# LuoweiZhou/VLP

Measured on NVIDIA H100. Metric: image_text_samples_per_sec, higher is better.
Workload: dtype bf16

## Files before the change

vlp_b200/csrc/api.cu:

```cuda
#include "../../include/vlpk.h"

#include <cstdlib>
#include <cstring>

#include "attn.cuh"
#include "gemm.cuh"
#include "head.cuh"
#include "host.cuh"
#include "optim.cuh"
#include "rowops.cuh"
#include "tables.cuh"

using namespace vlpk;
typedef __nv_bfloat16 bf16;

namespace {

inline cudaStream_t S(void* s) { return reinterpret_cast<cudaStream_t>(s); }

enum { SITE_ATTN = 0, SITE_HID1 = 1, SITE_HID2 = 2 };
inline uint64_t site_of(uint64_t layer_id, int site) { return layer_id * 8 + site; }

inline DropoutCfg mk_drop(const VlpkDropout* d, float p, uint64_t site) {
  if (d == nullptr || p <= 0.f) return make_dropout(0.f, 0, site);
// ... 324 lines not shown
    o[j] = pack_bf16x2(v.x > 0.f ? d.x * scale : 0.f, v.y > 0.f ? d.y * scale : 0.f);
  }
  *reinterpret_cast<uint4*>(dpre + i) = make_uint4(o[0], o[1], o[2], o[3]);
}

}

#pragma GCC visibility push(default)
extern "C" {

int vlpk_version(void) { return VLPK_VERSION; }
int vlpk_debug_set_option(const char* name, int value) {
  VLPK_CHECK_ARG(name != nullptr, "set_option: null name");
  if (strcmp(name, "wgrad_stream") == 0) { g_wgrad_stream = value ? 1 : 0; return 0; }
  if (strcmp(name, "attn_tiled") == 0) { set_attn_tiled(value != 0); return 0; }
  set_error("set_option: unknown option '%s'", name);
  return -1;
}
int vlpk_debug_plan_gemm(int M, int N, int K, int a_mn, int b_mn, int nseg, int seg_rows, int epi, int bn, int splits, int* out2) {
  GemmDesc g;
  g.M = M; g.N = N; g.K = K;
  g.a_mn = a_mn != 0; g.b_mn = b_mn != 0;
  g.nseg = nseg; g.b_seg_rows = seg_rows;
  g.epi = epi; g.bn = bn; g.splits = splits;
  return plan_gemm(g, &out2[0], &out2[1]);
}
void vlpk_set_reserved_sms(int n) { set_reserved_sms(n); }
void vlpk_set_deterministic(int on) { set_deterministic(on != 0); }
const char* vlpk_last_error(void) { return get_error(); }

// ... 405 lines not shown
```

vlp_b200/csrc/attn.cu:

```cuda
#include "attn.cuh"
#include "host.cuh"
#include "rowops.cuh"

namespace vlpk {

static constexpr int HD = 64;
static constexpr int TL = 128;
static constexpr int TILE_B = TL * 128;
static constexpr float LOG2E = 1.4426950408889634f;
static constexpr float LN2 = 0.6931471805599453f;
static constexpr int ATT_THREADS = 256;

struct AttnTmaps {
  CUtensorMap q, k, v, o;
  CUtensorMap dq, dk, dv;
};

struct AttnArgs {
  int B, heads, Lq, Lkv;
  const uint32_t* mask_bits;
  int mask_rows;
  float* lse;
  const __nv_bfloat16* o_ptr;
  const __nv_bfloat16* do_ptr;
// ... 13 lines not shown
    const int t = threadIdx.x & 127, lane = threadIdx.x & 31;
    fr = (t >> 5) * 16 + (lane >> 2);
    fc = (lane & 3) * 2;
  }
};

__device__ __forceinline__ float quad_max(float v) {
  v = fmaxf(v, __shfl_xor_sync(0xffffffffu, v, 1));
  return fmaxf(v, __shfl_xor_sync(0xffffffffu, v, 2));
}
__device__ __forceinline__ float quad_sum(float v) {
  v += __shfl_xor_sync(0xffffffffu, v, 1);
  return v + __shfl_xor_sync(0xffffffffu, v, 2);
}

__device__ __forceinline__ void attn_keep_words(const DropoutCfg& d, uint64_t dseed, const uint64_t (&row_elem0)[2], uint32_t (&kw)[2][4]) {
  const int lane = threadIdx.x & 31, qi = lane & 3;
#pragma unroll
  for (int h = 0; h < 2; ++h) {
    uint32_t mine = 0xFFFFFFFFu;
    if (d.p > 0.f) {
      if (d.bits != nullptr) {
        mine = __ldg(reinterpret_cast<const uint32_t*>(d.bits + (row_elem0[h] >> 3)) + qi);
      } else {
        mine = 0;
#pragma unroll
        for (int g = 0; g < 4; ++g) mine |= dropout_keep8(dseed, d.site, (row_elem0[h] + qi * 32 + g * 8) >> 3, d.thresh16) << (8 * g);
      }
    }
#pragma unroll
    for (int w = 0; w < 4; ++w) kw[h][w] = __shfl_sync(0xffffffffu, mine, (lane & ~3) | w);
  }
}

__device__ __forceinline__ float score(float s, const uint32_t (&mw)[4], int col, int Lkv) {
  const float x = s * (0.125f * LOG2E) + (((mw[col >> 5] >> (col & 31)) & 1u) ? 0.f : -10000.0f * LOG2E);
  return col < Lkv ? x : -INFINITY;
}

__device__ __forceinline__ void load_mask_words(const AttnArgs& a, int b, int row, uint32_t (&mw)[4]) {
  const int mr = (a.mask_rows == 1) ? 0 : min(row, a.mask_rows - 1);
  const uint4 m4 = __ldg(reinterpret_cast<const uint4*>(a.mask_bits + (static_cast<size_t>(b) * a.mask_rows + mr) * 4));
  mw[0] = m4.x; mw[1] = m4.y; mw[2] = m4.z; mw[3] = m4.w;
}

struct FwdSmem {
  static constexpr int OFF_Q = 0;
  static constexpr int OFF_K = TILE_B;
  static constexpr int OFF_V = 2 * TILE_B;
  static constexpr int OFF_BAR = 3 * TILE_B;
  static constexpr int TOTAL = OFF_BAR + 16;
  static constexpr int DYN = TOTAL + 1024;
};

__global__ void __launch_bounds__(ATT_THREADS, 2) attn_fwd_kernel(const __grid_constant__ AttnTmaps tm, const AttnArgs a) {
  extern __shared__ uint8_t smem_raw[];
  uint8_t* smem = reinterpret_cast<uint8_t*>((reinterpret_cast<uintptr_t>(smem_raw) + 1023) & ~uintptr_t(1023));
  uint8_t* sQ = smem + FwdSmem::OFF_Q;
  uint8_t* sK = smem + FwdSmem::OFF_K;
  uint8_t* sV = smem + FwdSmem::OFF_V;
  uint64_t* bars = reinterpret_cast<uint64_t*>(smem + FwdSmem::OFF_BAR);
  uint64_t* bar_qk = &bars[0];
  uint64_t* bar_v = &bars[1];

  pdl_launch_dependents();
  const int h = blockIdx.x, b = blockIdx.y;
  const int tid = threadIdx.x, wg = tid >> 7;
  const Frag f;
  const int qi = tid & 3;

  if (tid == 0) {
    tma_prefetch_desc(&tm.q);
    tma_prefetch_desc(&tm.k);
    tma_prefetch_desc(&tm.v);
    tma_prefetch_desc(&tm.o);
    mbar_init(bar_qk, 1);
    mbar_init(bar_v, 1);
    fence_mbar_init();
  }
  __syncthreads();
  pdl_wait();
  if (tid == 0) {
    mbar_arrive_expect_tx(bar_qk, 2 * TILE_B);
    tma_load_3d(sQ, &tm.q, bar_qk, h * HD, 0, b);
    tma_load_3d(sK, &tm.k, bar_qk, h * HD, 0, b);
    mbar_arrive_expect_tx(bar_v, TILE_B);
    tma_load_3d(sV, &tm.v, bar_v, h * HD, 0, b);
  }

  const int row[2] = {wg * 64 + f.fr, wg * 64 + f.fr + 8};
  uint32_t mw[2][4];
  uint64_t row_elem0[2];
#pragma unroll
  for (int hh = 0; hh < 2; ++hh) {
    load_mask_words(a, b, row[hh], mw[hh]);
    row_elem0[hh] = ((static_cast<uint64_t>(b) * a.heads + h) * a.Lq + min(row[hh], a.Lq - 1)) * TL;
  }

  float s[64];
  mbar_wait(bar_qk, 0);
  {
    const uint32_t q0 = smem_u32(sQ) + wg * 8192, k0 = smem_u32(sK);
    wgmma_fence();
#pragma unroll
    for (int k = 0; k < HD / 16; ++k)
      wgmma_m64n128k16_ss<0, 0>(s, wgmma_desc_sw128(q0 + k * 32, 16, 1024), wgmma_desc_sw128(k0 + k * 32, 16, 1024), k > 0 ? 1u : 0u);
    wgmma_commit();
    wgmma_wait<0>();
    reg_fence(s);
  }
  float mx[2] = {-INFINITY, -INFINITY};
#pragma unroll
  for (int i = 0; i < 64; ++i) {
    const int hh = (i >> 1) & 1;
    s[i] = score(s[i], mw[hh], 8 * (i >> 2) + f.fc + (i & 1), a.Lkv);
    mx[hh] = fmaxf(mx[hh], s[i]);
  }
  mx[0] = quad_max(mx[0]);
  mx[1] = quad_max(mx[1]);
  uint32_t kw[2][4];
  attn_keep_words(a.drop, drop_seed(a.drop), row_elem0, kw);
  if (a.keep_out != nullptr) {
#pragma unroll
    for (int hh = 0; hh < 2; ++hh)
      if (row[hh] < a.Lq) reinterpret_cast<uint32_t*>(a.keep_out + (row_elem0[hh] >> 3))[qi] = kw[hh][qi];
  }
  float rsum[2] = {0.f, 0.f}, lsum[2] = {0.f, 0.f};
  uint32_t pa[8][4];
#pragma unroll
  for (int i = 0; i < 64; i += 2) {
    const int hh = (i >> 1) & 1, col = 8 * (i >> 2) + f.fc;
    const float x0 = fast_ex2(s[i] - mx[hh]), x1 = fast_ex2(s[i + 1] - mx[hh]);
    lsum[hh] += x0 + x1;
    const float e0 = bf16_round(x0), e1 = bf16_round(x1);
    rsum[hh] += e0 + e1;
    const uint32_t keep = kw[hh][col >> 5] >> (col & 31);
    const float p0 = (keep & 1u) ? e0 * a.drop.scale : 0.f;
    const float p1 = (keep & 2u) ? e1 * a.drop.scale : 0.f;
    pa[i >> 3][(i >> 1) & 3] = pack_bf16x2(p0, p1);
  }
#pragma unroll
  for (int hh = 0; hh < 2; ++hh) {
    rsum[hh] = quad_sum(rsum[hh]);
    lsum[hh] = quad_sum(lsum[hh]);
    if (qi == 0 && a.lse != nullptr && row[hh] < a.Lq)
      a.lse[(static_cast<size_t>(b) * a.heads + h) * a.Lq + row[hh]] = (mx[hh] + log2f(lsum[hh])) * LN2;
  }
  float o[32];
  mbar_wait(bar_v, 0);
  {
    const uint32_t v0 = smem_u32(sV);
    wgmma_fence();
#pragma unroll
    for (int k = 0; k < TL / 16; ++k) wgmma_m64n64k16_rs<1>(o, pa[k], wgmma_desc_sw128(v0 + k * 2048, 8192, 1024), k > 0 ? 1u : 0u);
    wgmma_commit();
    wgmma_wait<0>();
    reg_fence(o);
  }
  const float inv[2] = {1.0f / rsum[0], 1.0f / rsum[1]};
  uint8_t* stg = sQ + wg * 8192;
#pragma unroll
  for (int i = 0; i < 32; i += 2) {
    const int hh = (i >> 1) & 1;
    sw_write_pair(stg, f.fr + 8 * hh, 8 * (i >> 2) + f.fc, pack_bf16x2(o[i] * inv[hh], o[i + 1] * inv[hh]));
  }
  fence_proxy_async_smem();
  __syncthreads();
  if (tid == 0) {
    tma_store_3d(&tm.o, sQ, h * HD, 0, b);
    tma_store_commit();
    tma_store_wait<0>();
  }
}

struct BwdSmem {
  static constexpr int OFF_Q = 0;
  static constexpr int OFF_K = TILE_B;
  static constexpr int OFF_V = 2 * TILE_B;
  static constexpr int OFF_DO = 3 * TILE_B;
  static constexpr int OFF_PD = 4 * TILE_B;
  static constexpr int OFF_BAR = 6 * TILE_B;
  static constexpr int TOTAL = OFF_BAR + 16;
  static constexpr int DYN = TOTAL + 1024;
};

__global__ void __launch_bounds__(ATT_THREADS, 1) attn_bwd_kernel(const __grid_constant__ AttnTmaps tm, const AttnArgs a) {
  extern __shared__ uint8_t smem_raw[];
  uint8_t* smem = reinterpret_cast<uint8_t*>((reinterpret_cast<uintptr_t>(smem_raw) + 1023) & ~uintptr_t(1023));
  uint8_t* sQ = smem + BwdSmem::OFF_Q;
  uint8_t* sK = smem + BwdSmem::OFF_K;
  uint8_t* sV = smem + BwdSmem::OFF_V;
  uint8_t* sdO = smem + BwdSmem::OFF_DO;
  uint8_t* sPD = smem + BwdSmem::OFF_PD;
  uint64_t* bar_in = reinterpret_cast<uint64_t*>(smem + BwdSmem::OFF_BAR);

  pdl_launch_dependents();
  const int h = blockIdx.x, b = blockIdx.y;
  const int tid = threadIdx.x, wg = tid >> 7;
  const Frag f;

  if (tid == 0) {
    tma_prefetch_desc(&tm.q);
    tma_prefetch_desc(&tm.k);
    tma_prefetch_desc(&tm.v);
    tma_prefetch_desc(&tm.o);
    mbar_init(bar_in, 1);
    fence_mbar_init();
  }
  __syncthreads();
  pdl_wait();
  if (tid == 0) {
    mbar_arrive_expect_tx(bar_in, 4 * TILE_B);
    tma_load_3d(sQ, &tm.q, bar_in, h * HD, 0, b);
    tma_load_3d(sK, &tm.k, bar_in, h * HD, 0, b);
    tma_load_3d(sV, &tm.v, bar_in, h * HD, 0, b);
    tma_load_3d(sdO, &tm.o, bar_in, h * HD, 0, b);
  }

  const int row[2] = {wg * 64 + f.fr, wg * 64 + f.fr + 8};
  uint32_t mw[2][4];
  uint64_t row_elem0[2];
  float lse2[2];
  bool row_ok[2];
#pragma unroll
  for (int hh = 0; hh < 2; ++hh) {
    load_mask_words(a, b, row[hh], mw[hh]);
    row_elem0[hh] = ((static_cast<uint64_t>(b) * a.heads + h) * a.Lq + min(row[hh], a.Lq - 1)) * TL;
    row_ok[hh] = row[hh] < a.Lq;
    lse2[hh] = row_ok[hh] ? a.lse[(static_cast<size_t>(b) * a.heads + h) * a.Lq + row[hh]] * LOG2E : 0.f;
  }
  uint32_t kw[2][4];
  attn_keep_words(a.drop, drop_seed(a.drop), row_elem0, kw);

  float s[64], dp[64];
  mbar_wait(bar_in, 0);
  {
    const uint32_t q0 = smem_u32(sQ) + wg * 8192, k0 = smem_u32(sK), do0 = smem_u32(sdO) + wg * 8192, v0 = smem_u32(sV);
    wgmma_fence();
#pragma unroll
    for (int k = 0; k < HD / 16; ++k)
      wgmma_m64n128k16_ss<0, 0>(s, wgmma_desc_sw128(q0 + k * 32, 16, 1024), wgmma_desc_sw128(k0 + k * 32, 16, 1024), k > 0 ? 1u : 0u);
#pragma unroll
    for (int k = 0; k < HD / 16; ++k)
      wgmma_m64n128k16_ss<0, 0>(dp, wgmma_desc_sw128(do0 + k * 32, 16, 1024), wgmma_desc_sw128(v0 + k * 32, 16, 1024), k > 0 ? 1u : 0u);
    wgmma_commit();
    wgmma_wait<0>();
    reg_fence(s);
    reg_fence(dp);
  }
  float delta[2] = {0.f, 0.f};
#pragma unroll
  for (int i = 0; i < 64; ++i) {
    const int hh = (i >> 1) & 1, col = 8 * (i >> 2) + f.fc + (i & 1);
    const float p = row_ok[hh] ? fast_ex2(score(s[i], mw[hh], col, a.Lkv) - lse2[hh]) : 0.f;
    const bool kp = (kw[hh][col >> 5] >> (col & 31)) & 1u;
    const float dpm = kp ? dp[i] * a.drop.scale : 0.f;
    delta[hh] = fmaf(p, dpm, delta[hh]);
    s[i] = p;
    dp[i] = dpm;
  }
  delta[0] = quad_sum(delta[0]);
  delta[1] = quad_sum(delta[1]);
  uint32_t dsa[8][4];
#pragma unroll
  for (int i = 0; i < 64; i += 2) {
    const int hh = (i >> 1) & 1, col = 8 * (i >> 2) + f.fc;
    const uint32_t keep = kw[hh][col >> 5] >> (col & 31);
    const float p0 = (keep & 1u) ? s[i] * a.drop.scale : 0.f, p1 = (keep & 2u) ? s[i + 1] * a.drop.scale : 0.f;
    sw_write_pair(sPD + (col >> 6) * TILE_B, row[hh], col & 63, pack_bf16x2(p0, p1));
    dsa[i >> 3][(i >> 1) & 3] = pack_bf16x2(s[i] * (dp[i] - delta[hh]) * 0.125f, s[i + 1] * (dp[i + 1] - delta[hh]) * 0.125f);
  }
  fence_proxy_async_smem();
  __syncthreads();

  float dv[32];
  {
    const uint32_t p0 = smem_u32(sPD) + wg * TILE_B, do0 = smem_u32(sdO);
    wgmma_fence();
#pragma unroll
    for (int k = 0; k < TL / 16; ++k)
      wgmma_m64n64k16_ss<1, 1>(dv, wgmma_desc_sw128(p0 + k * 2048, 8192, 1024), wgmma_desc_sw128(do0 + k * 2048, 8192, 1024), k > 0 ? 1u : 0u);
    wgmma_commit();
    wgmma_wait<0>();
    reg_fence(dv);
  }
  __syncthreads();
#pragma unroll
  for (int c = 0; c < 8; ++c)
#pragma unroll
    for (int e = 0; e < 4; ++e) {
      const int hh = e & 1, col = 16 * c + 8 * (e >> 1) + f.fc;
      sw_write_pair(sPD + (col >> 6) * TILE_B, row[hh], col & 63, dsa[c][e]);
    }
  fence_proxy_async_smem();
  __syncthreads();

  float dk[32], dq[32];
  {
    const uint32_t p0 = smem_u32(sPD) + wg * TILE_B, q0 = smem_u32(sQ), k0 = smem_u32(sK);
    wgmma_fence();
#pragma unroll
    for (int k = 0; k < TL / 16; ++k)
      wgmma_m64n64k16_ss<1, 1>(dk, wgmma_desc_sw128(p0 + k * 2048, 8192, 1024), wgmma_desc_sw128(q0 + k * 2048, 8192, 1024), k > 0 ? 1u : 0u);
#pragma unroll
    for (int k = 0; k < TL / 16; ++k) wgmma_m64n64k16_rs<1>(dq, dsa[k], wgmma_desc_sw128(k0 + k * 2048, 8192, 1024), k > 0 ? 1u : 0u);
    wgmma_commit();
    wgmma_wait<0>();
    reg_fence(dk);
    reg_fence(dq);
  }
  __syncthreads();
#pragma unroll
  for (int i = 0; i < 32; i += 2) {
    const int r = wg * 64 + f.fr + 8 * ((i >> 1) & 1), col = 8 * (i >> 2) + f.fc;
    sw_write_pair(sQ, r, col, pack_bf16x2(dq[i], dq[i + 1]));
    sw_write_pair(sK, r, col, pack_bf16x2(dk[i], dk[i + 1]));
    sw_write_pair(sV, r, col, pack_bf16x2(dv[i], dv[i + 1]));
  }
  fence_proxy_async_smem();
  __syncthreads();
  if (tid == 0) {
    tma_store_3d(&tm.dq, sQ, h * HD, 0, b);
    tma_store_3d(&tm.dk, sK, h * HD, 0, b);
    tma_store_3d(&tm.dv, sV, h * HD, 0, b);
    tma_store_commit();
  }
  if (a.dbias_part != nullptr && tid < 192) {
    const int o = tid >> 6, c = tid & 63;
    const uint8_t* stg = (o == 0) ? sQ : (o == 1 ? sK : sV);
    float acc = 0.f;
#pragma unroll 8
    for (int r = 0; r < TL; ++r)
      acc += __bfloat162float(*reinterpret_cast<const __nv_bfloat16*>(stg + r * 128 + (((c >> 3) ^ (r & 7)) << 4) + (c & 7) * 2));
    a.dbias_part[static_cast<size_t>(b) * 3 * a.heads * HD + o * a.heads * HD + h * HD + c] = acc;
  }
  if (tid == 0) tma_store_wait<0>();
}

static constexpr int MAX_SLOTS = 512;
static bool g_attn_tiled = false;

void set_attn_tiled(bool on) { g_attn_tiled = on; }

struct AttnTiledArgs {
  int B, heads, Lq, Lkv;
  int slots;
  int tiles;
  const uint32_t* mask_bits;
  int mask_rows;
  float* lse;
// ... 1 lines not shown
  DropoutCfg drop;
  unsigned char* keep_out;
  float* dbias_part;
};

__device__ __forceinline__ void load_mask_tile(const AttnTiledArgs& a, int b, int row, int kt, uint32_t (&mw)[4]) {
  const int mr = (a.mask_rows == 1) ? 0 : min(row, a.mask_rows - 1);
  const uint4 m4 = __ldg(reinterpret_cast<const uint4*>(a.mask_bits + (static_cast<size_t>(b) * a.mask_rows + mr) * (a.slots >> 5)) + kt);
  mw[0] = m4.x; mw[1] = m4.y; mw[2] = m4.z; mw[3] = m4.w;
}

__device__ __forceinline__ uint64_t tiled_row_elem0(const AttnTiledArgs& a, int b, int h, int row) {
  return ((static_cast<uint64_t>(b) * a.heads + h) * a.Lq + min(row, a.Lq - 1)) * a.slots;
}

__device__ __forceinline__ float staged_colsum(const uint8_t* stg, int c) {
  float acc = 0.f;
#pragma unroll 8
  for (int r = 0; r < TL; ++r)
    acc += __bfloat162float(*reinterpret_cast<const __nv_bfloat16*>(stg + r * 128 + (((c >> 3) ^ (r & 7)) << 4) + (c & 7) * 2));
  return acc;
}

struct FwdTiledSmem {
  static constexpr int OFF_Q = 0;
  static constexpr int OFF_KV = TILE_B;
  static constexpr int OFF_BAR = 5 * TILE_B;
  static constexpr int TOTAL = OFF_BAR + 24;
  static constexpr int DYN = TOTAL + 1024;
};

__global__ void __launch_bounds__(ATT_THREADS, 1) attn_fwd_tiled_kernel(const __grid_constant__ AttnTmaps tm, const AttnTiledArgs a) {
  extern __shared__ uint8_t smem_raw[];
  uint8_t* smem = reinterpret_cast<uint8_t*>((reinterpret_cast<uintptr_t>(smem_raw) + 1023) & ~uintptr_t(1023));
  uint8_t* sQ = smem + FwdTiledSmem::OFF_Q;
  uint8_t* sKV = smem + FwdTiledSmem::OFF_KV;
  uint64_t* bars = reinterpret_cast<uint64_t*>(smem + FwdTiledSmem::OFF_BAR);

// ... 426 lines not shown
  if (d.kv_slots == 0) {
    VLPK_CHECK_ARG(d.Lq >= 1 && d.Lq <= TL && d.Lkv >= 1 && d.Lkv <= TL, "attention: Lq=%d Lkv=%d must be in [1,128]",
                   d.Lq, d.Lkv);
  } else {
    VLPK_CHECK_ARG(d.Lkv >= 1 && d.Lkv <= MAX_SLOTS && d.kv_slots == (d.Lkv + TL - 1) / TL * TL && d.Lq >= 1 && d.Lq <= d.kv_slots,
                   "attention: Lq=%d Lkv=%d kv_slots=%d (needs Lkv in [1,512], kv_slots = 128 * ceil(Lkv / 128), Lq in [1,kv_slots])",
                   d.Lq, d.Lkv, d.kv_slots);
  }
  VLPK_CHECK_ARG(d.B >= 1 && d.heads >= 1, "attention: B=%d heads=%d", d.B, d.heads);
  VLPK_CHECK_ARG(d.mask_bits != nullptr && (d.mask_rows == 1 || d.mask_rows == d.Lq), "attention: mask rows %d",
                 d.mask_rows);
  return 0;
}

static bool use_tiled(const AttnDesc& d) { return g_attn_tiled || d.Lq > TL || d.Lkv > TL; }

static AttnTiledArgs tiled_args(const AttnDesc& d) {
  AttnTiledArgs a;
  a.B = d.B; a.heads = d.heads; a.Lq = d.Lq; a.Lkv = d.Lkv;
  a.slots = d.kv_slots != 0 ? d.kv_slots : TL;
  a.tiles = (d.Lq + TL - 1) / TL;
  a.mask_bits = d.mask_bits; a.mask_rows = d.mask_rows;
  a.lse = d.lse; a.delta = nullptr;
  a.drop = d.drop;
  a.keep_out = nullptr;
  a.dbias_part = nullptr;
  return a;
}

static int launch_attn_fwd_tiled(const AttnDesc& d, const AttnTmaps& tm, cudaStream_t stream) {
// ... 44 lines not shown
  AttnTmaps tm;
  memset(&tm, 0, sizeof(tm));
  VLPK_TRY(make_seq_tmap(&tm.q, d.q, width, d.Lq, d.B, d.ld_q));
  VLPK_TRY(make_seq_tmap(&tm.k, d.k, width, d.Lkv, d.B, d.ld_kv, d.kv_batch_stride));
  VLPK_TRY(make_seq_tmap(&tm.v, d.v, width, d.Lkv, d.B, d.ld_kv, d.kv_batch_stride));
  VLPK_TRY(make_seq_tmap(&tm.o, d.o, width, d.Lq, d.B, d.ld_o));
  tm.dq = tm.dk = tm.dv = tm.o;
  if (use_tiled(d)) return launch_attn_fwd_tiled(d, tm, stream);
  AttnArgs a;
  a.B = d.B; a.heads = d.heads; a.Lq = d.Lq; a.Lkv = d.Lkv;
  a.mask_bits = d.mask_bits; a.mask_rows = d.mask_rows;
  a.lse = d.lse; a.o_ptr = nullptr; a.do_ptr = nullptr; a.ld_o = d.ld_o;
  a.drop = d.drop;
  a.keep_out = d.keep_out;
  a.dbias_part = nullptr;
  static bool attr_set = false;
  if (!attr_set) {
    VLPK_CUDA(cudaFuncSetAttribute(attn_fwd_kernel, cudaFuncAttributeMaxDynamicSharedMemorySize, FwdSmem::DYN));
    attr_set = true;
  }
  LaunchScope scope(CAT_ATTN_FWD, 4.0 * d.B * d.heads * d.Lq * d.Lkv * HD, stream);
  VLPK_CUDA(launch_ex(attn_fwd_kernel, dim3(d.heads, d.B), dim3(ATT_THREADS), FwdSmem::DYN, stream, 1, tm, a));
  return 0;
}

int launch_attn_bwd(const AttnDesc& d, cudaStream_t stream) {
  VLPK_TRY(check_common(d));
  VLPK_CHECK_ARG(d.Lq == d.Lkv, "attention bwd: Lq must equal Lkv (training path)");
  VLPK_CHECK_ARG(d.lse != nullptr && d.d_o != nullptr && d.dq && d.dk && d.dv, "attention bwd: missing buffers");
  const int width = d.heads * HD;
  AttnTmaps tm;
  memset(&tm, 0, sizeof(tm));
  VLPK_TRY(make_seq_tmap(&tm.q, d.q, width, d.Lq, d.B, d.ld_q));
  VLPK_TRY(make_seq_tmap(&tm.k, d.k, width, d.Lkv, d.B, d.ld_kv));
  VLPK_TRY(make_seq_tmap(&tm.v, d.v, width, d.Lkv, d.B, d.ld_kv));
  VLPK_TRY(make_seq_tmap(&tm.o, d.d_o, width, d.Lq, d.B, d.ld_o));
  VLPK_TRY(make_seq_tmap(&tm.dq, d.dq, width, d.Lq, d.B, d.ld_dqkv));
// ... 3 lines not shown
  AttnArgs a;
  a.B = d.B; a.heads = d.heads; a.Lq = d.Lq; a.Lkv = d.Lkv;
  a.mask_bits = d.mask_bits; a.mask_rows = d.mask_rows;
  a.lse = d.lse;
  a.o_ptr = reinterpret_cast<const __nv_bfloat16*>(d.o);
  a.do_ptr = reinterpret_cast<const __nv_bfloat16*>(d.d_o);
  a.ld_o = d.ld_o;
  a.drop = d.drop;
  a.keep_out = nullptr;
  a.dbias_part = nullptr;
  const long long nbias = 3LL * d.heads * HD;
  if (d.dbias != nullptr) {
    a.dbias_part = scratch_f32(SCRATCH_ATTN_DBIAS, static_cast<size_t>(d.B) * nbias, stream);
    if (a.dbias_part == nullptr) return -1;
  }
  static bool attr_set = false;
  if (!attr_set) {
    VLPK_CUDA(cudaFuncSetAttribute(attn_bwd_kernel, cudaFuncAttributeMaxDynamicSharedMemorySize, BwdSmem::DYN));
    attr_set = true;
  }
  {
    LaunchScope scope(CAT_ATTN_BWD, 10.0 * d.B * d.heads * d.Lq * d.Lkv * HD, stream);
    VLPK_CUDA(launch_ex(attn_bwd_kernel, dim3(d.heads, d.B), dim3(ATT_THREADS), BwdSmem::DYN, stream, 1, tm, a));
  }
  if (d.dbias != nullptr) VLPK_TRY(launch_sum_parts(a.dbias_part, d.B, nbias, d.dbias, stream));
  return 0;
}

}
```

vlp_b200/csrc/attn.cuh:

```cuda
#pragma once
#include "common.cuh"

namespace vlpk {

struct AttnDesc {
  int B = 0, heads = 0, head_dim = 64;
  int Lq = 0, Lkv = 0;
  int kv_slots = 0;
  const void* q = nullptr;
  const void* k = nullptr;
  const void* v = nullptr;
  int64_t ld_q = 0, ld_kv = 0;
  int64_t kv_batch_stride = 0;
  void* o = nullptr;
  int64_t ld_o = 0;
  const uint32_t* mask_bits = nullptr;
  int mask_rows = 0;
  float* lse = nullptr;
  DropoutCfg drop = {0.f, 1.f, 0u, 0ull, 0ull, nullptr};
  unsigned char* keep_out = nullptr;
  const void* d_o = nullptr;
  void* dq = nullptr;
  void* dk = nullptr;
  void* dv = nullptr;
  int64_t ld_dqkv = 0;
  float* dbias = nullptr;
};

int launch_attn_fwd(const AttnDesc& d, cudaStream_t stream);
int launch_attn_bwd(const AttnDesc& d, cudaStream_t stream);
void set_attn_tiled(bool on);

}
```

Measured before the change: 4040.

## Make short-sequence attention kernels persistent with double-buffered TMA prefetch

Converts the single-tile attention forward and backward kernels from one CTA per (head, batch) into persistent CTAs sized by occupancy. Each CTA loops over work items and prefetches the next item's Q/K/V(/dO) via TMA into a second stage while computing the current one. The backward pass also overlaps the dbias column sums and the next item's mask/LSE/dropout loads with WGMMA, and mask bit extraction is precomputed with per-fragment shifts. The cost is that the forward shared memory doubles, which may lower occupancy, and the backward kernel adds a separate output staging area.

```diff
diff --git a/vlp_b200/csrc/api.cu b/vlp_b200/csrc/api.cu
--- a/vlp_b200/csrc/api.cu
+++ b/vlp_b200/csrc/api.cu
@@ -362,6 +362,7 @@
   VLPK_CHECK_ARG(name != nullptr, "set_option: null name");
   if (strcmp(name, "wgrad_stream") == 0) { g_wgrad_stream = value ? 1 : 0; return 0; }
   if (strcmp(name, "attn_tiled") == 0) { set_attn_tiled(value != 0); return 0; }
+  if (strcmp(name, "attn_ctas") == 0) { set_attn_ctas(value); return 0; }
   set_error("set_option: unknown option '%s'", name);
   return -1;
 }
diff --git a/vlp_b200/csrc/attn.cu b/vlp_b200/csrc/attn.cu
--- a/vlp_b200/csrc/attn.cu
+++ b/vlp_b200/csrc/attn.cu
@@ -51,29 +51,48 @@
   return v + __shfl_xor_sync(0xffffffffu, v, 2);
 }
 
-__device__ __forceinline__ void attn_keep_words(const DropoutCfg& d, uint64_t dseed, const uint64_t (&row_elem0)[2], uint32_t (&kw)[2][4]) {
-  const int lane = threadIdx.x & 31, qi = lane & 3;
+__device__ __forceinline__ void attn_keep_own(const DropoutCfg& d, uint64_t dseed, const uint64_t (&row_elem0)[2], uint32_t (&mine)[2]) {
+  const int qi = threadIdx.x & 3;
 #pragma unroll
   for (int h = 0; h < 2; ++h) {
-    uint32_t mine = 0xFFFFFFFFu;
+    mine[h] = 0xFFFFFFFFu;
     if (d.p > 0.f) {
       if (d.bits != nullptr) {
-        mine = __ldg(reinterpret_cast<const uint32_t*>(d.bits + (row_elem0[h] >> 3)) + qi);
+        mine[h] = __ldg(reinterpret_cast<const uint32_t*>(d.bits + (row_elem0[h] >> 3)) + qi);
       } else {
-        mine = 0;
-#pragma unroll
-        for (int g = 0; g < 4; ++g) mine |= dropout_keep8(dseed, d.site, (row_elem0[h] + qi * 32 + g * 8) >> 3, d.thresh16) << (8 * g);
+        mine[h] = 0;
+#pragma unroll
+        for (int g = 0; g < 4; ++g) mine[h] |= dropout_keep8(dseed, d.site, (row_elem0[h] + qi * 32 + g * 8) >> 3, d.thresh16) << (8 * g);
       }
     }
-#pragma unroll
-    for (int w = 0; w < 4; ++w) kw[h][w] = __shfl_sync(0xffffffffu, mine, (lane & ~3) | w);
-  }
-}
-
+  }
+}
+__device__ __forceinline__ void attn_keep_share(const uint32_t (&mine)[2], uint32_t (&kw)[2][4]) {
+  const int lane = threadIdx.x & 31;
+#pragma unroll
+  for (int h = 0; h < 2; ++h)
+#pragma unroll
+    for (int w = 0; w < 4; ++w) kw[h][w] = __shfl_sync(0xffffffffu, mine[h], (lane & ~3) | w);
+}
+__device__ __forceinline__ void attn_keep_words(const DropoutCfg& d, uint64_t dseed, const uint64_t (&row_elem0)[2], uint32_t (&kw)[2][4]) {
+  uint32_t mine[2];
+  attn_keep_own(d, dseed, row_elem0, mine);
+  attn_keep_share(mine, kw);
+}
+
+__device__ __forceinline__ float score_bit(float s, uint32_t attend, bool valid) {
+  const float x = s * (0.125f * LOG2E) + (attend ? 0.f : -10000.0f * LOG2E);
+  return valid ? x : -INFINITY;
+}
 __device__ __forceinline__ float score(float s, const uint32_t (&mw)[4], int col, int Lkv) {
-  const float x = s * (0.125f * LOG2E) + (((mw[col >> 5] >> (col & 31)) & 1u) ? 0.f : -10000.0f * LOG2E);
-  return col < Lkv ? x : -INFINITY;
-}
+  return score_bit(s, (mw[col >> 5] >> (col & 31)) & 1u, col < Lkv);
+}
+
+__device__ __forceinline__ void frag_shift(uint32_t (&w)[4], int fc) {
+#pragma unroll
+  for (int j = 0; j < 4; ++j) w[j] >>= fc;
+}
+__device__ __forceinline__ uint32_t frag_bit(const uint32_t (&w)[4], int i) { return (w[i >> 4] >> (8 * ((i >> 2) & 3) + (i & 1))) & 1u; }
 
 __device__ __forceinline__ void load_mask_words(const AttnArgs& a, int b, int row, uint32_t (&mw)[4]) {
   const int mr = (a.mask_rows == 1) ? 0 : min(row, a.mask_rows - 1);
@@ -81,296 +100,349 @@
   mw[0] = m4.x; mw[1] = m4.y; mw[2] = m4.z; mw[3] = m4.w;
 }
 
+static int g_attn_ctas = 0;
+
+void set_attn_ctas(int n) { g_attn_ctas = n > 0 ? n : 0; }
+
 struct FwdSmem {
-  static constexpr int OFF_Q = 0;
-  static constexpr int OFF_K = TILE_B;
-  static constexpr int OFF_V = 2 * TILE_B;
-  static constexpr int OFF_BAR = 3 * TILE_B;
-  static constexpr int TOTAL = OFF_BAR + 16;
+  static constexpr int STAGE = 3 * TILE_B;
+  static constexpr int OFF_BAR = 2 * STAGE;
+  static constexpr int TOTAL = OFF_BAR + 32;
   static constexpr int DYN = TOTAL + 1024;
 };
 
 __global__ void __launch_bounds__(ATT_THREADS, 2) attn_fwd_kernel(const __grid_constant__ AttnTmaps tm, const AttnArgs a) {
   extern __shared__ uint8_t smem_raw[];
   uint8_t* smem = reinterpret_cast<uint8_t*>((reinterpret_cast<uintptr_t>(smem_raw) + 1023) & ~uintptr_t(1023));
-  uint8_t* sQ = smem + FwdSmem::OFF_Q;
-  uint8_t* sK = smem + FwdSmem::OFF_K;
-  uint8_t* sV = smem + FwdSmem::OFF_V;
   uint64_t* bars = reinterpret_cast<uint64_t*>(smem + FwdSmem::OFF_BAR);
-  uint64_t* bar_qk = &bars[0];
-  uint64_t* bar_v = &bars[1];
 
   pdl_launch_dependents();
-  const int h = blockIdx.x, b = blockIdx.y;
   const int tid = threadIdx.x, wg = tid >> 7;
   const Frag f;
   const int qi = tid & 3;
+
+  auto load_item = [&](int w, int st) {
+    const int h = w % a.heads, b = w / a.heads;
+    uint8_t* sq = smem + st * FwdSmem::STAGE;
+    mbar_arrive_expect_tx(&bars[2 * st], 2 * TILE_B);
+    tma_load_3d(sq, &tm.q, &bars[2 * st], h * HD, 0, b);
+    tma_load_3d(sq + TILE_B, &tm.k, &bars[2 * st], h * HD, 0, b);
+    mbar_arrive_expect_tx(&bars[2 * st + 1], TILE_B);
+    tma_load_3d(sq + 2 * TILE_B, &tm.v, &bars[2 * st + 1], h * HD, 0, b);
+  };
 
   if (tid == 0) {
     tma_prefetch_desc(&tm.q);
     tma_prefetch_desc(&tm.k);
     tma_prefetch_desc(&tm.v);
     tma_prefetch_desc(&tm.o);
-    mbar_init(bar_qk, 1);
-    mbar_init(bar_v, 1);
+    for (int i = 0; i < 4; ++i) mbar_init(&bars[i], 1);
     fence_mbar_init();
   }
   __syncthreads();
   pdl_wait();
-  if (tid == 0) {
-    mbar_arrive_expect_tx(bar_qk, 2 * TILE_B);
-    tma_load_3d(sQ, &tm.q, bar_qk, h * HD, 0, b);
-    tma_load_3d(sK, &tm.k, bar_qk, h * HD, 0, b);
-    mbar_arrive_expect_tx(bar_v, TILE_B);
-    tma_load_3d(sV, &tm.v, bar_v, h * HD, 0, b);
-  }
+  if (tid == 0) load_item(blockIdx.x, 0);
 
   const int row[2] = {wg * 64 + f.fr, wg * 64 + f.fr + 8};
-  uint32_t mw[2][4];
-  uint64_t row_elem0[2];
-#pragma unroll
-  for (int hh = 0; hh < 2; ++hh) {
-    load_mask_words(a, b, row[hh], mw[hh]);
-    row_elem0[hh] = ((static_cast<uint64_t>(b) * a.heads + h) * a.Lq + min(row[hh], a.Lq - 1)) * TL;
-  }
-
-  float s[64];
-  mbar_wait(bar_qk, 0);
-  {
-    const uint32_t q0 = smem_u32(sQ) + wg * 8192, k0 = smem_u32(sK);
-    wgmma_fence();
-#pragma unroll
-    for (int k = 0; k < HD / 16; ++k)
-      wgmma_m64n128k16_ss<0, 0>(s, wgmma_desc_sw128(q0 + k * 32, 16, 1024), wgmma_desc_sw128(k0 + k * 32, 16, 1024), k > 0 ? 1u : 0u);
-    wgmma_commit();
+  int it = 0;
+  for (int w = blockIdx.x; w < a.B * a.heads; w += gridDim.x, ++it) {
+    const int st = it & 1;
+    const uint32_t par = (it >> 1) & 1;
+    const int h = w % a.heads, b = w / a.heads;
+    uint8_t* sQ = smem + st * FwdSmem::STAGE;
+    if (tid == 0 && w + static_cast<int>(gridDim.x) < a.B * a.heads) {
+      tma_store_wait_read<0>();
+      load_item(w + gridDim.x, st ^ 1);
+    }
+
+    uint32_t mw[2][4];
+#pragma unroll
+    for (int hh = 0; hh < 2; ++hh) {
+      load_mask_words(a, b, row[hh], mw[hh]);
+      frag_shift(mw[hh], f.fc);
+    }
+
+    float s[64];
+    mbar_wait(&bars[2 * st], par);
+    {
+      const uint32_t q0 = smem_u32(sQ) + wg * 8192, k0 = smem_u32(sQ + TILE_B);
+      wgmma_fence();
+#pragma unroll
+      for (int k = 0; k < HD / 16; ++k)
+        wgmma_m64n128k16_ss<0, 0>(s, wgmma_desc_sw128(q0 + k * 32, 16, 1024), wgmma_desc_sw128(k0 + k * 32, 16, 1024), k > 0 ? 1u : 0u);
+      wgmma_commit();
+    }
+    uint64_t row_elem0[2];
+#pragma unroll
+    for (int hh = 0; hh < 2; ++hh) row_elem0[hh] = (static_cast<uint64_t>(w) * a.Lq + min(row[hh], a.Lq - 1)) * TL;
+    uint32_t mine[2];
+    attn_keep_own(a.drop, drop_seed(a.drop), row_elem0, mine);
     wgmma_wait<0>();
     reg_fence(s);
-  }
-  float mx[2] = {-INFINITY, -INFINITY};
-#pragma unroll
-  for (int i = 0; i < 64; ++i) {
-    const int hh = (i >> 1) & 1;
-    s[i] = score(s[i], mw[hh], 8 * (i >> 2) + f.fc + (i & 1), a.Lkv);
-    mx[hh] = fmaxf(mx[hh], s[i]);
-  }
-  mx[0] = quad_max(mx[0]);
-  mx[1] = quad_max(mx[1]);
-  uint32_t kw[2][4];
-  attn_keep_words(a.drop, drop_seed(a.drop), row_elem0, kw);
-  if (a.keep_out != nullptr) {
-#pragma unroll
-    for (int hh = 0; hh < 2; ++hh)
-      if (row[hh] < a.Lq) reinterpret_cast<uint32_t*>(a.keep_out + (row_elem0[hh] >> 3))[qi] = kw[hh][qi];
-  }
-  float rsum[2] = {0.f, 0.f}, lsum[2] = {0.f, 0.f};
-  uint32_t pa[8][4];
-#pragma unroll
-  for (int i = 0; i < 64; i += 2) {
-    const int hh = (i >> 1) & 1, col = 8 * (i >> 2) + f.fc;
-    const float x0 = fast_ex2(s[i] - mx[hh]), x1 = fast_ex2(s[i + 1] - mx[hh]);
-    lsum[hh] += x0 + x1;
-    const float e0 = bf16_round(x0), e1 = bf16_round(x1);
-    rsum[hh] += e0 + e1;
-    const uint32_t keep = kw[hh][col >> 5] >> (col & 31);
-    const float p0 = (keep & 1u) ? e0 * a.drop.scale : 0.f;
-    const float p1 = (keep & 2u) ? e1 * a.drop.scale : 0.f;
-    pa[i >> 3][(i >> 1) & 3] = pack_bf16x2(p0, p1);
-  }
-#pragma unroll
-  for (int hh = 0; hh < 2; ++hh) {
-    rsum[hh] = quad_sum(rsum[hh]);
-    lsum[hh] = quad_sum(lsum[hh]);
-    if (qi == 0 && a.lse != nullptr && row[hh] < a.Lq)
-      a.lse[(static_cast<size_t>(b) * a.heads + h) * a.Lq + row[hh]] = (mx[hh] + log2f(lsum[hh])) * LN2;
-  }
-  float o[32];
-  mbar_wait(bar_v, 0);
-  {
-    const uint32_t v0 = smem_u32(sV);
-    wgmma_fence();
-#pragma unroll
-    for (int k = 0; k < TL / 16; ++k) wgmma_m64n64k16_rs<1>(o, pa[k], wgmma_desc_sw128(v0 + k * 2048, 8192, 1024), k > 0 ? 1u : 0u);
-    wgmma_commit();
-    wgmma_wait<0>();
-    reg_fence(o);
-  }
-  const float inv[2] = {1.0f / rsum[0], 1.0f / rsum[1]};
-  uint8_t* stg = sQ + wg * 8192;
-#pragma unroll
-  for (int i = 0; i < 32; i += 2) {
-    const int hh = (i >> 1) & 1;
-    sw_write_pair(stg, f.fr + 8 * hh, 8 * (i >> 2) + f.fc, pack_bf16x2(o[i] * inv[hh], o[i + 1] * inv[hh]));
-  }
-  fence_proxy_async_smem();
-  __syncthreads();
-  if (tid == 0) {
-    tma_store_3d(&tm.o, sQ, h * HD, 0, b);
-    tma_store_commit();
-    tma_store_wait<0>();
-  }
+    float mx[2] = {-INFINITY, -INFINITY};
+    const int lim = a.Lkv - f.fc;
+#pragma unroll
+    for (int i = 0; i < 64; ++i) {
+      const int hh = (i >> 1) & 1;
+      s[i] = score_bit(s[i], frag_bit(mw[hh], i), 8 * (i >> 2) + (i & 1) < lim);
+      mx[hh] = fmaxf(mx[hh], s[i]);
+    }
+    mx[0] = quad_max(mx[0]);
+    mx[1] = quad_max(mx[1]);
+    uint32_t kw[2][4];
+    attn_keep_share(mine, kw);
+    frag_shift(kw[0], f.fc);
+    frag_shift(kw[1], f.fc);
+    if (a.keep_out != nullptr) {
+#pragma unroll
+      for (int hh = 0; hh < 2; ++hh)
+        if (row[hh] < a.Lq) reinterpret_cast<uint32_t*>(a.keep_out + (row_elem0[hh] >> 3))[qi] = mine[hh];
+    }
+    float rsum[2] = {0.f, 0.f}, lsum[2] = {0.f, 0.f};
+    uint32_t pa[8][4];
+#pragma unroll
+    for (int i = 0; i < 64; i += 2) {
+      const int hh = (i >> 1) & 1;
+      const float x0 = fast_ex2(s[i] - mx[hh]), x1 = fast_ex2(s[i + 1] - mx[hh]);
+      lsum[hh] += x0 + x1;
+      const float e0 = bf16_round(x0), e1 = bf16_round(x1);
+      rsum[hh] += e0 + e1;
+      const float p0 = frag_bit(kw[hh], i) ? e0 * a.drop.scale : 0.f;
+      const float p1 = frag_bit(kw[hh], i + 1) ? e1 * a.drop.scale : 0.f;
+      pa[i >> 3][(i >> 1) & 3] = pack_bf16x2(p0, p1);
+    }
+#pragma unroll
+    for (int hh = 0; hh < 2; ++hh) {
+      rsum[hh] = quad_sum(rsum[hh]);
+      lsum[hh] = quad_sum(lsum[hh]);
+      if (qi == 0 && a.lse != nullptr && row[hh] < a.Lq)
+        a.lse[static_cast<size_t>(w) * a.Lq + row[hh]] = (mx[hh] + log2f(lsum[hh])) * LN2;
+    }
+    float o[32];
+    mbar_wait(&bars[2 * st + 1], par);
+    {
+      const uint32_t v0 = smem_u32(sQ + 2 * TILE_B);
+      wgmma_fence();
+#pragma unroll
+      for (int k = 0; k < TL / 16; ++k) wgmma_m64n64k16_rs<1>(o, pa[k], wgmma_desc_sw128(v0 + k * 2048, 8192, 1024), k > 0 ? 1u : 0u);
+      wgmma_commit();
+      wgmma_wait<0>();
+      reg_fence(o);
+    }
+    const float inv[2] = {1.0f / rsum[0], 1.0f / rsum[1]};
+    uint8_t* stg = sQ + wg * 8192;
+#pragma unroll
+    for (int i = 0; i < 32; i += 2) {
+      const int hh = (i >> 1) & 1;
+      sw_write_pair(stg, f.fr + 8 * hh, 8 * (i >> 2) + f.fc, pack_bf16x2(o[i] * inv[hh], o[i + 1] * inv[hh]));
+    }
+    fence_proxy_async_smem();
+    __syncthreads();
+    if (tid == 0) {
+      tma_store_3d(&tm.o, sQ, h * HD, 0, b);
+      tma_store_commit();
+    }
+  }
+  if (tid == 0) tma_store_wait<0>();
 }
 
 struct BwdSmem {
-  static constexpr int OFF_Q = 0;
-  static constexpr int OFF_K = TILE_B;
-  static constexpr int OFF_V = 2 * TILE_B;
-  static constexpr int OFF_DO = 3 * TILE_B;
-  static constexpr int OFF_PD = 4 * TILE_B;
-  static constexpr int OFF_BAR = 6 * TILE_B;
+  static constexpr int STAGE = 4 * TILE_B;
+  static constexpr int OFF_PD = 2 * STAGE;
+  static constexpr int OFF_STG = OFF_PD + 2 * TILE_B;
+  static constexpr int OFF_BAR = OFF_STG + 3 * TILE_B;
   static constexpr int TOTAL = OFF_BAR + 16;
   static constexpr int DYN = TOTAL + 1024;
 };
 
+__device__ __forceinline__ float staged_colsum(const uint8_t* stg, int c) {
+  float acc = 0.f;
+#pragma unroll 8
+  for (int r = 0; r < TL; ++r)
+    acc += __bfloat162float(*reinterpret_cast<const __nv_bfloat16*>(stg + r * 128 + (((c >> 3) ^ (r & 7)) << 4) + (c & 7) * 2));
+  return acc;
+}
+
+struct BwdRows {
+  uint32_t mw[2][4];
+  float lse2[2];
+  uint32_t keep[2];
+};
+
+__device__ __forceinline__ void load_bwd_rows(const AttnArgs& a, uint64_t dseed, int w, const int (&row)[2], BwdRows& r) {
+  const int b = w / a.heads;
+  uint64_t row_elem0[2];
+#pragma unroll
+  for (int hh = 0; hh < 2; ++hh) {
+    load_mask_words(a, b, row[hh], r.mw[hh]);
+    frag_shift(r.mw[hh], Frag().fc);
+    row_elem0[hh] = (static_cast<uint64_t>(w) * a.Lq + min(row[hh], a.Lq - 1)) * TL;
+    r.lse2[hh] = row[hh] < a.Lq ? a.lse[static_cast<size_t>(w) * a.Lq + row[hh]] * LOG2E : INFINITY;
+  }
+  attn_keep_own(a.drop, dseed, row_elem0, r.keep);
+}
+
 __global__ void __launch_bounds__(ATT_THREADS, 1) attn_bwd_kernel(const __grid_constant__ AttnTmaps tm, const AttnArgs a) {
   extern __shared__ uint8_t smem_raw[];
   uint8_t* smem = reinterpret_cast<uint8_t*>((reinterpret_cast<uintptr_t>(smem_raw) + 1023) & ~uintptr_t(1023));
-  uint8_t* sQ = smem + BwdSmem::OFF_Q;
-  uint8_t* sK = smem + BwdSmem::OFF_K;
-  uint8_t* sV = smem + BwdSmem::OFF_V;
-  uint8_t* sdO = smem + BwdSmem::OFF_DO;
   uint8_t* sPD = smem + BwdSmem::OFF_PD;
-  uint64_t* bar_in = reinterpret_cast<uint64_t*>(smem + BwdSmem::OFF_BAR);
+  uint8_t* sdQ = smem + BwdSmem::OFF_STG;
+  uint8_t* sdK = sdQ + TILE_B;
+  uint8_t* sdV = sdQ + 2 * TILE_B;
+  uint64_t* bars = reinterpret_cast<uint64_t*>(smem + BwdSmem::OFF_BAR);
 
   pdl_launch_dependents();
-  const int h = blockIdx.x, b = blockIdx.y;
   const int tid = threadIdx.x, wg = tid >> 7;
   const Frag f;
+  const int items = a.B * a.heads;
+
+  auto load_item = [&](int w, int st) {
+    const int h = w % a.heads, b = w / a.heads;
+    uint8_t* sq = smem + st * BwdSmem::STAGE;
+    mbar_arrive_expect_tx(&bars[st], 4 * TILE_B);
+    tma_load_3d(sq, &tm.q, &bars[st], h * HD, 0, b);
+    tma_load_3d(sq + TILE_B, &tm.k, &bars[st], h * HD, 0, b);
+    tma_load_3d(sq + 2 * TILE_B, &tm.v, &bars[st], h * HD, 0, b);
+    tma_load_3d(sq + 3 * TILE_B, &tm.o, &bars[st], h * HD, 0, b);
+  };
+  auto store_bias_part = [&](int w) {
+    if (a.dbias_part != nullptr && tid < 3 * HD) {
+      const int h = w % a.heads, b = w / a.heads, o = tid >> 6, c = tid & 63;
+      a.dbias_part[static_cast<size_t>(b) * 3 * a.heads * HD + o * a.heads * HD + h * HD + c] = staged_colsum(sdQ + o * TILE_B, c);
+    }
+  };
 
   if (tid == 0) {
     tma_prefetch_desc(&tm.q);
     tma_prefetch_desc(&tm.k);
     tma_prefetch_desc(&tm.v);
     tma_prefetch_desc(&tm.o);
-    mbar_init(bar_in, 1);
+    mbar_init(&bars[0], 1);
+    mbar_init(&bars[1], 1);
     fence_mbar_init();
   }
   __syncthreads();
   pdl_wait();
-  if (tid == 0) {
-    mbar_arrive_expect_tx(bar_in, 4 * TILE_B);
-    tma_load_3d(sQ, &tm.q, bar_in, h * HD, 0, b);
-    tma_load_3d(sK, &tm.k, bar_in, h * HD, 0, b);
-    tma_load_3d(sV, &tm.v, bar_in, h * HD, 0, b);
-    tma_load_3d(sdO, &tm.o, bar_in, h * HD, 0, b);
-  }
-
+  if (tid == 0) load_item(blockIdx.x, 0);
+
+  const uint64_t dseed = drop_seed(a.drop);
   const int row[2] = {wg * 64 + f.fr, wg * 64 + f.fr + 8};
-  uint32_t mw[2][4];
-  uint64_t row_elem0[2];
-  float lse2[2];
-  bool row_ok[2];
-#pragma unroll
-  for (int hh = 0; hh < 2; ++hh) {
-    load_mask_words(a, b, row[hh], mw[hh]);
-    row_elem0[hh] = ((static_cast<uint64_t>(b) * a.heads + h) * a.Lq + min(row[hh], a.Lq - 1)) * TL;
-    row_ok[hh] = row[hh] < a.Lq;
-    lse2[hh] = row_ok[hh] ? a.lse[(static_cast<size_t>(b) * a.heads + h) * a.Lq + row[hh]] * LOG2E : 0.f;
-  }
-  uint32_t kw[2][4];
-  attn_keep_words(a.drop, drop_seed(a.drop), row_elem0, kw);
-
-  float s[64], dp[64];
-  mbar_wait(bar_in, 0);
-  {
-    const uint32_t q0 = smem_u32(sQ) + wg * 8192, k0 = smem_u32(sK), do0 = smem_u32(sdO) + wg * 8192, v0 = smem_u32(sV);
-    wgmma_fence();
-#pragma unroll
-    for (int k = 0; k < HD / 16; ++k)
-      wgmma_m64n128k16_ss<0, 0>(s, wgmma_desc_sw128(q0 + k * 32, 16, 1024), wgmma_desc_sw128(k0 + k * 32, 16, 1024), k > 0 ? 1u : 0u);
-#pragma unroll
-    for (int k = 0; k < HD / 16; ++k)
-      wgmma_m64n128k16_ss<0, 0>(dp, wgmma_desc_sw128(do0 + k * 32, 16, 1024), wgmma_desc_sw128(v0 + k * 32, 16, 1024), k > 0 ? 1u : 0u);
-    wgmma_commit();
-    wgmma_wait<0>();
-    reg_fence(s);
-    reg_fence(dp);
-  }
-  float delta[2] = {0.f, 0.f};
-#pragma unroll
-  for (int i = 0; i < 64; ++i) {
-    const int hh = (i >> 1) & 1, col = 8 * (i >> 2) + f.fc + (i & 1);
-    const float p = row_ok[hh] ? fast_ex2(score(s[i], mw[hh], col, a.Lkv) - lse2[hh]) : 0.f;
-    const bool kp = (kw[hh][col >> 5] >> (col & 31)) & 1u;
-    const float dpm = kp ? dp[i] * a.drop.scale : 0.f;
-    delta[hh] = fmaf(p, dpm, delta[hh]);
-    s[i] = p;
-    dp[i] = dpm;
-  }
-  delta[0] = quad_sum(delta[0]);
-  delta[1] = quad_sum(delta[1]);
-  uint32_t dsa[8][4];
-#pragma unroll
-  for (int i = 0; i < 64; i += 2) {
-    const int hh = (i >> 1) & 1, col = 8 * (i >> 2) + f.fc;
-    const uint32_t keep = kw[hh][col >> 5] >> (col & 31);
-    const float p0 = (keep & 1u) ? s[i] * a.drop.scale : 0.f, p1 = (keep & 2u) ? s[i + 1] * a.drop.scale : 0.f;
-    sw_write_pair(sPD + (col >> 6) * TILE_B, row[hh], col & 63, pack_bf16x2(p0, p1));
-    dsa[i >> 3][(i >> 1) & 3] = pack_bf16x2(s[i] * (dp[i] - delta[hh]) * 0.125f, s[i + 1] * (dp[i + 1] - delta[hh]) * 0.125f);
-  }
-  fence_proxy_async_smem();
-  __syncthreads();
-
-  float dv[32];
-  {
-    const uint32_t p0 = smem_u32(sPD) + wg * TILE_B, do0 = smem_u32(sdO);
-    wgmma_fence();
-#pragma unroll
-    for (int k = 0; k < TL / 16; ++k)
-      wgmma_m64n64k16_ss<1, 1>(dv, wgmma_desc_sw128(p0 + k * 2048, 8192, 1024), wgmma_desc_sw128(do0 + k * 2048, 8192, 1024), k > 0 ? 1u : 0u);
-    wgmma_commit();
-    wgmma_wait<0>();
-    reg_fence(dv);
-  }
-  __syncthreads();
-#pragma unroll
-  for (int c = 0; c < 8; ++c)
-#pragma unroll
-    for (int e = 0; e < 4; ++e) {
-      const int hh = e & 1, col = 16 * c + 8 * (e >> 1) + f.fc;
-      sw_write_pair(sPD + (col >> 6) * TILE_B, row[hh], col & 63, dsa[c][e]);
-    }
-  fence_proxy_async_smem();
-  __syncthreads();
-
-  float dk[32], dq[32];
-  {
-    const uint32_t p0 = smem_u32(sPD) + wg * TILE_B, q0 = smem_u32(sQ), k0 = smem_u32(sK);
-    wgmma_fence();
-#pragma unroll
-    for (int k = 0; k < TL / 16; ++k)
-      wgmma_m64n64k16_ss<1, 1>(dk, wgmma_desc_sw128(p0 + k * 2048, 8192, 1024), wgmma_desc_sw128(q0 + k * 2048, 8192, 1024), k > 0 ? 1u : 0u);
-#pragma unroll
-    for (int k = 0; k < TL / 16; ++k) wgmma_m64n64k16_rs<1>(dq, dsa[k], wgmma_desc_sw128(k0 + k * 2048, 8192, 1024), k > 0 ? 1u : 0u);
-    wgmma_commit();
-    wgmma_wait<0>();
-    reg_fence(dk);
-    reg_fence(dq);
-  }
-  __syncthreads();
-#pragma unroll
-  for (int i = 0; i < 32; i += 2) {
-    const int r = wg * 64 + f.fr + 8 * ((i >> 1) & 1), col = 8 * (i >> 2) + f.fc;
-    sw_write_pair(sQ, r, col, pack_bf16x2(dq[i], dq[i + 1]));
-    sw_write_pair(sK, r, col, pack_bf16x2(dk[i], dk[i + 1]));
-    sw_write_pair(sV, r, col, pack_bf16x2(dv[i], dv[i + 1]));
-  }
-  fence_proxy_async_smem();
-  __syncthreads();
-  if (tid == 0) {
-    tma_store_3d(&tm.dq, sQ, h * HD, 0, b);
-    tma_store_3d(&tm.dk, sK, h * HD, 0, b);
-    tma_store_3d(&tm.dv, sV, h * HD, 0, b);
-    tma_store_commit();
-  }
-  if (a.dbias_part != nullptr && tid < 192) {
-    const int o = tid >> 6, c = tid & 63;
-    const uint8_t* stg = (o == 0) ? sQ : (o == 1 ? sK : sV);
-    float acc = 0.f;
-#pragma unroll 8
-    for (int r = 0; r < TL; ++r)
-      acc += __bfloat162float(*reinterpret_cast<const __nv_bfloat16*>(stg + r * 128 + (((c >> 3) ^ (r & 7)) << 4) + (c & 7) * 2));
-    a.dbias_part[static_cast<size_t>(b) * 3 * a.heads * HD + o * a.heads * HD + h * HD + c] = acc;
-  }
+  const int lim = a.Lkv - f.fc;
+  BwdRows nxt;
+  load_bwd_rows(a, dseed, blockIdx.x, row, nxt);
+  int it = 0, prev = -1;
+  for (int w = blockIdx.x; w < items; prev = w, w += gridDim.x, ++it) {
+    const int st = it & 1;
+    const int h = w % a.heads, b = w / a.heads;
+    const bool more = w + static_cast<int>(gridDim.x) < items;
+    uint8_t* sQ = smem + st * BwdSmem::STAGE;
+    uint8_t* sK = sQ + TILE_B;
+    uint8_t* sV = sQ + 2 * TILE_B;
+    uint8_t* sdO = sQ + 3 * TILE_B;
+    if (tid == 0 && more) load_item(w + gridDim.x, st ^ 1);
+
+    const BwdRows cur = nxt;
+    uint32_t kw[2][4];
+    attn_keep_share(cur.keep, kw);
+    frag_shift(kw[0], f.fc);
+    frag_shift(kw[1], f.fc);
+
+    float s[64], dp[64];
+    mbar_wait(&bars[st], (it >> 1) & 1);
+    {
+      const uint32_t q0 = smem_u32(sQ) + wg * 8192, k0 = smem_u32(sK), do0 = smem_u32(sdO) + wg * 8192, v0 = smem_u32(sV);
+      wgmma_fence();
+#pragma unroll
+      for (int k = 0; k < HD / 16; ++k)
+        wgmma_m64n128k16_ss<0, 0>(s, wgmma_desc_sw128(q0 + k * 32, 16, 1024), wgmma_desc_sw128(k0 + k * 32, 16, 1024), k > 0 ? 1u : 0u);
+#pragma unroll
+      for (int k = 0; k < HD / 16; ++k)
+        wgmma_m64n128k16_ss<0, 0>(dp, wgmma_desc_sw128(do0 + k * 32, 16, 1024), wgmma_desc_sw128(v0 + k * 32, 16, 1024), k > 0 ? 1u : 0u);
+      wgmma_commit();
+      if (prev >= 0) store_bias_part(prev);
+      wgmma_wait<0>();
+      reg_fence(s);
+      reg_fence(dp);
+    }
+    float delta[2] = {0.f, 0.f};
+#pragma unroll
+    for (int i = 0; i < 64; ++i) {
+      const int hh = (i >> 1) & 1;
+      const float p = fast_ex2(score_bit(s[i], frag_bit(cur.mw[hh], i), 8 * (i >> 2) + (i & 1) < lim) - cur.lse2[hh]);
+      const float dpm = frag_bit(kw[hh], i) ? dp[i] * a.drop.scale : 0.f;
+      delta[hh] = fmaf(p, dpm, delta[hh]);
+      s[i] = p;
+      dp[i] = dpm;
+    }
+    delta[0] = quad_sum(delta[0]);
+    delta[1] = quad_sum(delta[1]);
+    uint32_t dsa[8][4];
+#pragma unroll
+    for (int i = 0; i < 64; i += 2) {
+      const int hh = (i >> 1) & 1, col = 8 * (i >> 2) + f.fc;
+      const float p0 = frag_bit(kw[hh], i) ? s[i] * a.drop.scale : 0.f, p1 = frag_bit(kw[hh], i + 1) ? s[i + 1] * a.drop.scale : 0.f;
+      sw_write_pair(sPD + (col >> 6) * TILE_B, row[hh], col & 63, pack_bf16x2(p0, p1));
+      dsa[i >> 3][(i >> 1) & 3] = pack_bf16x2(s[i] * (dp[i] - delta[hh]) * 0.125f, s[i + 1] * (dp[i + 1] - delta[hh]) * 0.125f);
+    }
+    fence_proxy_async_smem();
+    __syncthreads();
+
+    float dv[32];
+    {
+      const uint32_t p0 = smem_u32(sPD) + wg * TILE_B, do0 = smem_u32(sdO);
+      wgmma_fence();
+#pragma unroll
+      for (int k = 0; k < TL / 16; ++k)
+        wgmma_m64n64k16_ss<1, 1>(dv, wgmma_desc_sw128(p0 + k * 2048, 8192, 1024), wgmma_desc_sw128(do0 + k * 2048, 8192, 1024), k > 0 ? 1u : 0u);
+      wgmma_commit();
+      wgmma_wait<0>();
+      reg_fence(dv);
+    }
+    __syncthreads();
+#pragma unroll
+    for (int c = 0; c < 8; ++c)
+#pragma unroll
+      for (int e = 0; e < 4; ++e) {
+        const int hh = e & 1, col = 16 * c + 8 * (e >> 1) + f.fc;
+        sw_write_pair(sPD + (col >> 6) * TILE_B, row[hh], col & 63, dsa[c][e]);
+      }
+    fence_proxy_async_smem();
+    __syncthreads();
+
+    float dk[32], dq[32];
+    {
+      const uint32_t p0 = smem_u32(sPD) + wg * TILE_B, q0 = smem_u32(sQ), k0 = smem_u32(sK);
+      wgmma_fence();
+#pragma unroll
+      for (int k = 0; k < TL / 16; ++k)
+        wgmma_m64n64k16_ss<1, 1>(dk, wgmma_desc_sw128(p0 + k * 2048, 8192, 1024), wgmma_desc_sw128(q0 + k * 2048, 8192, 1024), k > 0 ? 1u : 0u);
+#pragma unroll
+      for (int k = 0; k < TL / 16; ++k) wgmma_m64n64k16_rs<1>(dq, dsa[k], wgmma_desc_sw128(k0 + k * 2048, 8192, 1024), k > 0 ? 1u : 0u);
+      wgmma_commit();
+      if (more) load_bwd_rows(a, dseed, w + gridDim.x, row, nxt);
+      wgmma_wait<0>();
+      reg_fence(dk);
+      reg_fence(dq);
+    }
+    if (tid == 0) tma_store_wait_read<0>();
+    __syncthreads();
+#pragma unroll
+    for (int i = 0; i < 32; i += 2) {
+      const int r = wg * 64 + f.fr + 8 * ((i >> 1) & 1), col = 8 * (i >> 2) + f.fc;
+      sw_write_pair(sdQ, r, col, pack_bf16x2(dq[i], dq[i + 1]));
+      sw_write_pair(sdK, r, col, pack_bf16x2(dk[i], dk[i + 1]));
+      sw_write_pair(sdV, r, col, pack_bf16x2(dv[i], dv[i + 1]));
+    }
+    fence_proxy_async_smem();
+    __syncthreads();
+    if (tid == 0) {
+      tma_store_3d(&tm.dq, sdQ, h * HD, 0, b);
+      tma_store_3d(&tm.dk, sdK, h * HD, 0, b);
+      tma_store_3d(&tm.dv, sdV, h * HD, 0, b);
+      tma_store_commit();
+    }
+  }
+  if (prev >= 0) store_bias_part(prev);
   if (tid == 0) tma_store_wait<0>();
 }
 
@@ -402,14 +474,6 @@
   return ((static_cast<uint64_t>(b) * a.heads + h) * a.Lq + min(row, a.Lq - 1)) * a.slots;
 }
 
-__device__ __forceinline__ float staged_colsum(const uint8_t* stg, int c) {
-  float acc = 0.f;
-#pragma unroll 8
-  for (int r = 0; r < TL; ++r)
-    acc += __bfloat162float(*reinterpret_cast<const __nv_bfloat16*>(stg + r * 128 + (((c >> 3) ^ (r & 7)) << 4) + (c & 7) * 2));
-  return acc;
-}
-
 struct FwdTiledSmem {
   static constexpr int OFF_Q = 0;
   static constexpr int OFF_KV = TILE_B;
@@ -866,6 +930,12 @@
 }
 
 static bool use_tiled(const AttnDesc& d) { return g_attn_tiled || d.Lq > TL || d.Lkv > TL; }
+
+static int attn_grid(int items, int per_sm) {
+  int n = (per_sm > 0 ? per_sm : 1) * gemm_sms();
+  if (g_attn_ctas > 0 && g_attn_ctas < n) n = g_attn_ctas;
+  return n < items ? n : items;
+}
 
 static AttnTiledArgs tiled_args(const AttnDesc& d) {
   AttnTiledArgs a;
@@ -940,13 +1010,13 @@
   a.drop = d.drop;
   a.keep_out = d.keep_out;
   a.dbias_part = nullptr;
-  static bool attr_set = false;
-  if (!attr_set) {
+  static int per_sm = 0;
+  if (per_sm == 0) {
     VLPK_CUDA(cudaFuncSetAttribute(attn_fwd_kernel, cudaFuncAttributeMaxDynamicSharedMemorySize, FwdSmem::DYN));
-    attr_set = true;
+    VLPK_CUDA(cudaOccupancyMaxActiveBlocksPerMultiprocessor(&per_sm, attn_fwd_kernel, ATT_THREADS, FwdSmem::DYN));
   }
   LaunchScope scope(CAT_ATTN_FWD, 4.0 * d.B * d.heads * d.Lq * d.Lkv * HD, stream);
-  VLPK_CUDA(launch_ex(attn_fwd_kernel, dim3(d.heads, d.B), dim3(ATT_THREADS), FwdSmem::DYN, stream, 1, tm, a));
+  VLPK_CUDA(launch_ex(attn_fwd_kernel, dim3(attn_grid(d.B * d.heads, per_sm)), dim3(ATT_THREADS), FwdSmem::DYN, stream, 1, tm, a));
   return 0;
 }
 
@@ -980,14 +1050,14 @@
     a.dbias_part = scratch_f32(SCRATCH_ATTN_DBIAS, static_cast<size_t>(d.B) * nbias, stream);
     if (a.dbias_part == nullptr) return -1;
   }
-  static bool attr_set = false;
-  if (!attr_set) {
+  static int per_sm = 0;
+  if (per_sm == 0) {
     VLPK_CUDA(cudaFuncSetAttribute(attn_bwd_kernel, cudaFuncAttributeMaxDynamicSharedMemorySize, BwdSmem::DYN));
-    attr_set = true;
+    VLPK_CUDA(cudaOccupancyMaxActiveBlocksPerMultiprocessor(&per_sm, attn_bwd_kernel, ATT_THREADS, BwdSmem::DYN));
   }
   {
     LaunchScope scope(CAT_ATTN_BWD, 10.0 * d.B * d.heads * d.Lq * d.Lkv * HD, stream);
-    VLPK_CUDA(launch_ex(attn_bwd_kernel, dim3(d.heads, d.B), dim3(ATT_THREADS), BwdSmem::DYN, stream, 1, tm, a));
+    VLPK_CUDA(launch_ex(attn_bwd_kernel, dim3(attn_grid(d.B * d.heads, per_sm)), dim3(ATT_THREADS), BwdSmem::DYN, stream, 1, tm, a));
   }
   if (d.dbias != nullptr) VLPK_TRY(launch_sum_parts(a.dbias_part, d.B, nbias, d.dbias, stream));
   return 0;
diff --git a/vlp_b200/csrc/attn.cuh b/vlp_b200/csrc/attn.cuh
--- a/vlp_b200/csrc/attn.cuh
+++ b/vlp_b200/csrc/attn.cuh
@@ -30,5 +30,6 @@
 int launch_attn_fwd(const AttnDesc& d, cudaStream_t stream);
 int launch_attn_bwd(const AttnDesc& d, cudaStream_t stream);
 void set_attn_tiled(bool on);
+void set_attn_ctas(int n);
 
 }
```

Result: faster. 4127, median of 6 (+2.2%).
